# ddcr/shape_based_matching

Measured on AMD Instinct MI355X. Metric: templates*Mpixels/sec (whole Detector::match, frame resident in HBM), higher is better.
Workload: dtype u8; 1 GPU; case1 on MI355X: 1024x1024x3 frames x 360 templates per GPU (131/71 features), pyramid T={4,8}, threshold 90, 16 frame(s) per step, every frame's match list gathered to the host every step; stage=whole Detector::match per frame, templates_total=360, templates_per_gpu=360, parallelism=template-shard x1, frames_in_flight=64, input_buffers=8, exchange=none, n_ranks_seen=1, matches_distinct=8

## Files before the change

include/sbm.h:

```cpp
#ifndef SBM_H
#define SBM_H

#include <stdint.h>
#include "sbm_types.h"

#ifdef __cplusplus
extern "C" {
#endif

#define SBM_ABI_VERSION 1

typedef enum sbm_status {
    SBM_OK = 0,
    SBM_ERR_INVALID = -1,
    SBM_ERR_HIP = -2,
    SBM_ERR_CAPACITY = -3,
    SBM_ERR_STATE = -4
} sbm_status;

typedef struct sbm_ctx sbm_ctx;

typedef struct sbm_config {
    int32_t n_levels;
    int32_t T[SBM_MAX_LEVELS];
// ... 96 lines not shown
int64_t sbm_canonicalize(sbm_match_rec* recs, int64_t n);

typedef struct sbm_nms_params {
    float score_threshold;
    float nms_threshold;
    float eta;
    int32_t top_k;
} sbm_nms_params;
int sbm_nms_batch_device(sbm_ctx* ctx, const void* d_recs, const void* d_counts, int64_t cap, int32_t n_frames,
                         int32_t n_parts, int64_t part_stride, const sbm_nms_params* p, void* d_out, int64_t out_cap,
                         void* d_out_counts, void* stream);
int sbm_match_batch_host_end_nms(sbm_ctx* ctx, const sbm_nms_params* p, sbm_match_rec* out, int64_t out_cap, int32_t* counts);

int sbm_build_pyramid(sbm_ctx* ctx, const uint8_t* img_host, int32_t rows, int32_t cols,
                      int32_t stride, int32_t channels, const uint8_t* mask_host);
int sbm_set_quantized(sbm_ctx* ctx, int32_t level, const uint8_t* quantized_host, int32_t rows,
                      int32_t cols);
int sbm_get_quantized(sbm_ctx* ctx, int32_t level, uint8_t* out_host);
int sbm_get_quantized_frame(sbm_ctx* ctx, int32_t level, int32_t frame, uint8_t* out_host);
int sbm_get_linear_memories(sbm_ctx* ctx, int32_t level, uint8_t* out_host, int64_t cap_bytes,
                            int64_t* lm_stride);
int sbm_get_coarse_bitplanes(sbm_ctx* ctx, int32_t frame, uint8_t* out_host, int64_t cap_bytes);
int sbm_get_coarse_form(sbm_ctx* ctx, int32_t out[4]);
int sbm_level_dims(sbm_ctx* ctx, int32_t level, int32_t* rows, int32_t* cols);

int sbm_match_templates(sbm_ctx* ctx, float threshold, sbm_match_rec* out_host, int64_t cap,
                        int64_t* n_out);

int sbm_match_templates_device(sbm_ctx* ctx, float threshold, void* d_out, int64_t cap, void* d_count,
                               void* stream);


int sbm_quantized_orientations(sbm_ctx* ctx, const uint8_t* img_host, int32_t rows, int32_t cols,
                               int32_t stride, int32_t channels, float weak_threshold,
                               float* magnitude, uint8_t* angle, float* angle_ori);
int sbm_extract_local_maxima(sbm_ctx* ctx, const float* magnitude_host, const uint8_t* mask_host, int32_t rows, int32_t cols,
                             float strong_threshold, int32_t* xy, int64_t cap, int64_t* n_out);
int sbm_orientation_bins(sbm_ctx* ctx, const int16_t* gx, const int16_t* gy, int64_t n, uint8_t* q16);
int sbm_resize_linear(sbm_ctx* ctx, const uint8_t* img_host, int32_t rows, int32_t cols, int32_t stride, int32_t channels,
                      double fx, double fy, uint8_t* out, int64_t cap_bytes, int32_t* out_rows, int32_t* out_cols);
int sbm_pyrdown(sbm_ctx* ctx, const uint8_t* img_host, int32_t rows, int32_t cols, int32_t stride,
                int32_t channels, uint8_t* out_host);
int sbm_spread(sbm_ctx* ctx, const uint8_t* src_host, int32_t rows, int32_t cols, int32_t T,
               uint8_t* dst_host);
int sbm_compute_response_maps(sbm_ctx* ctx, const uint8_t* spread_host, int32_t rows, int32_t cols,
                              uint8_t* maps_host);
// ... 31 lines not shown
```

shape_based_matching_amd/capi.py:

```python
from __future__ import annotations

import ctypes as C
import os
from typing import List, Optional, Sequence, Tuple

import numpy as np

from .templates import FEATURE_DTYPE, LEVEL_DTYPE, MATCH_DTYPE, TemplateSet

TRAIN_FEATURE_DTYPE = np.dtype([("x", "<i4"), ("y", "<i4"), ("label", "<i4"), ("theta", "<f4")])

_HERE = os.path.dirname(os.path.abspath(__file__))
LIB_PATH = os.path.join(_HERE, "libsbm_hip.so")
SBM_MAX_LEVELS = 8

ABI_SYMBOLS = [
    "sbm_last_error", "sbm_abi_version", "sbm_create", "sbm_destroy", "sbm_upload_templates",
    "sbm_select_classes", "sbm_select_range", "sbm_match", "sbm_match_device", "sbm_match_batch_device", "sbm_canonicalize",
    "sbm_build_pyramid", "sbm_set_quantized", "sbm_get_quantized", "sbm_get_linear_memories",
    "sbm_level_dims", "sbm_match_templates", "sbm_quantized_orientations", "sbm_pyrdown", "sbm_spread",
    "sbm_compute_response_maps", "sbm_linearize", "sbm_similarity", "sbm_similarity_local",
    "sbm_set_profiling", "sbm_get_timings", "sbm_coarse_bytes", "sbm_get_stats",
    "sbm_set_result_mirror", "sbm_set_graph_mode", "sbm_set_quantize_mode", "sbm_resize_linear",
    "sbm_match_templates_device", "sbm_orientation_bins",
    "sbm_comm_unique_id", "sbm_comm_init", "sbm_comm_destroy", "sbm_match_device_sharded", "sbm_match_batch_device_sharded",
    "sbm_match_batch_device_banded", "sbm_pin_host_buffer", "sbm_unpin_host_buffer",
    "sbm_select_templates", "sbm_partition_templates", "sbm_match_sharded",
    "sbm_match_batch_host", "sbm_match_batch_host_begin", "sbm_match_batch_host_end", "sbm_extract_local_maxima",
    "sbm_train_batch", "sbm_train_batch_device",
    "sbm_set_pipeline_depth", "sbm_set_coarse_mode", "sbm_set_refine_order", "sbm_set_refine_bits", "sbm_get_coarse_bitplanes",
    "sbm_comm_count", "sbm_match_templates_device_sharded", "sbm_graph_count",
    "sbm_nms_batch_device", "sbm_match_batch_host_end_nms",
    "sbm_match_batch_device_masked", "sbm_match_batch_host_begin_masked", "sbm_match_batch_host_masked", "sbm_get_quantized_frame",
    "sbm_get_coarse_form",
]


class SbmConfig(C.Structure):
    _fields_ = [
        ("n_levels", C.c_int32),
        ("T", C.c_int32 * SBM_MAX_LEVELS),
        ("weak_threshold", C.c_float),
        ("device_id", C.c_int32),
        ("max_candidates", C.c_int64),
    ]


class SbmNmsParams(C.Structure):
    _fields_ = [
        ("score_threshold", C.c_float),
        ("nms_threshold", C.c_float),
        ("eta", C.c_float),
        ("top_k", C.c_int32),
    ]


class SbmError(RuntimeError):
# ... 84 lines not shown
    L.sbm_last_error.restype = C.c_char_p
    L.sbm_abi_version.restype = i32
    L.sbm_create.argtypes = [C.POINTER(SbmConfig), C.POINTER(vp)]
    L.sbm_destroy.argtypes = [vp]
    L.sbm_destroy.restype = None
    L.sbm_upload_templates.argtypes = [vp, i32, vp, vp, i64, vp, vp]
    L.sbm_select_classes.argtypes = [vp, vp, i32]
    L.sbm_select_range.argtypes = [vp, i32, i32]
    L.sbm_match.argtypes = [vp, vp, i32, i32, i32, i32, vp, f32, vp, i64, C.POINTER(i64)]
    L.sbm_match_device.argtypes = [vp, vp, i32, i32, i32, i32, vp, f32, vp, i64, vp, vp]
    L.sbm_match_batch_device.argtypes = [vp, vp, i64, i32, i32, i32, i32, i32, vp, f32, vp, i64, vp, vp]
    L.sbm_match_batch_device_masked.argtypes = [vp, vp, i64, i32, i32, i32, i32, i32, vp, i64, f32, vp, i64, vp, vp]
    L.sbm_match_batch_host_begin_masked.argtypes = [vp, vp, i32, i32, i32, i32, i32, vp, f32, i64, i32]
    L.sbm_match_batch_host_masked.argtypes = [vp, vp, i32, i32, i32, i32, i32, vp, f32, vp, i64, vp, i32]
    L.sbm_get_quantized_frame.argtypes = [vp, i32, i32, vp]
    L.sbm_canonicalize.argtypes = [vp, i64]
    L.sbm_canonicalize.restype = i64
    L.sbm_build_pyramid.argtypes = [vp, vp, i32, i32, i32, i32, vp]
    L.sbm_set_quantized.argtypes = [vp, i32, vp, i32, i32]
    L.sbm_get_quantized.argtypes = [vp, i32, vp]
    L.sbm_get_linear_memories.argtypes = [vp, i32, vp, i64, C.POINTER(i64)]
    L.sbm_get_coarse_bitplanes.argtypes = [vp, i32, vp, i64]
    L.sbm_get_coarse_form.argtypes = [vp, vp]
    L.sbm_level_dims.argtypes = [vp, i32, C.POINTER(i32), C.POINTER(i32)]
    L.sbm_match_templates.argtypes = [vp, f32, vp, i64, C.POINTER(i64)]
    L.sbm_quantized_orientations.argtypes = [vp, vp, i32, i32, i32, i32, f32, vp, vp, vp]
    L.sbm_pyrdown.argtypes = [vp, vp, i32, i32, i32, i32, vp]
    L.sbm_orientation_bins.argtypes = [vp, vp, vp, i64, vp]
    L.sbm_spread.argtypes = [vp, vp, i32, i32, i32, vp]
    L.sbm_compute_response_maps.argtypes = [vp, vp, i32, i32, vp]
    L.sbm_linearize.argtypes = [vp, vp, i32, i32, i32, vp]
    L.sbm_similarity.argtypes = [vp, i32, vp]
    L.sbm_similarity_local.argtypes = [vp, i32, i32, i32, i32, vp]
    L.sbm_set_profiling.argtypes = [vp, i32]
    L.sbm_get_timings.argtypes = [vp, vp, vp, i32, C.POINTER(i32)]
    L.sbm_coarse_bytes.argtypes = [vp, C.POINTER(i64)]
    L.sbm_get_stats.argtypes = [vp, C.POINTER(i64), C.POINTER(i64)]
    L.sbm_set_result_mirror.argtypes = [vp, vp, vp]
    L.sbm_set_graph_mode.argtypes = [vp, i32]
    L.sbm_graph_count.argtypes = [vp, C.POINTER(i32)]
    L.sbm_set_quantize_mode.argtypes = [vp, i32, i32]
    L.sbm_resize_linear.argtypes = [vp, vp, i32, i32, i32, i32, C.c_double, C.c_double, vp, i64, C.POINTER(i32), C.POINTER(i32)]
    L.sbm_match_templates_device.argtypes = [vp, f32, vp, i64, vp, vp]
    L.sbm_comm_unique_id.argtypes = [vp]
    L.sbm_comm_init.argtypes = [vp, i32, i32, vp]
    L.sbm_comm_count.argtypes = [vp, C.POINTER(i32)]
# ... 375 lines not shown
        out = np.empty((r, c), np.uint8)
        _check(lib().sbm_get_quantized_frame(self._h, level, frame, _p(out)))
        return out

    def get_linear_memories(self, level: int) -> np.ndarray:
        s = C.c_int64()
        _check(lib().sbm_get_linear_memories(self._h, level, None, 0, C.byref(s)))
        out = np.empty((8, s.value), np.uint8)
        _check(lib().sbm_get_linear_memories(self._h, level, _p(out), out.nbytes, C.byref(s)))
        return out

    def get_coarse_bitplanes(self, frame: int = 0) -> np.ndarray:
        s = C.c_int64()
        _check(lib().sbm_get_linear_memories(self._h, self.n_levels - 1, None, 0, C.byref(s)))
        out = np.empty((16, s.value // 8), np.uint8)
        _check(lib().sbm_get_coarse_bitplanes(self._h, frame, _p(out), out.nbytes))
        return out

    def coarse_form(self) -> Tuple[int, int, int, int]:
        out = np.zeros(4, np.int32)
        _check(lib().sbm_get_coarse_form(self._h, _p(out)))
        return tuple(int(v) for v in out)

    def match_templates(self, threshold: float) -> np.ndarray:
        out = np.empty(self._cap, MATCH_DTYPE)
        n = C.c_int64(0)
        _check(lib().sbm_match_templates(self._h, C.c_float(threshold), _p(out), self._cap, C.byref(n)))
        return out[: n.value].copy()

    def match_templates_device(self, threshold: float, d_out: int, cap: int, d_count: int, stream: int = 0):
        _check(lib().sbm_match_templates_device(self._h, C.c_float(threshold), C.c_void_p(d_out), cap, C.c_void_p(d_count),
                                                C.c_void_p(stream) if stream else None))

    def quantized_orientations(self, img: np.ndarray, weak: float, want_float: bool = True):
        img, r, c, ch = _img(img)
        ang = np.empty((r, c), np.uint8)
        mag = np.empty((r, c), np.float32) if want_float else None
        ori = np.empty((r, c), np.float32) if want_float else None
        _check(lib().sbm_quantized_orientations(self._h, _p(img), r, c, c * ch, ch, C.c_float(weak), _p(mag), _p(ang), _p(ori)))
        return mag, ang, ori

    def orientation_bins(self, gx: np.ndarray, gy: np.ndarray) -> np.ndarray:
        gx = np.ascontiguousarray(gx, np.int16)
        gy = np.ascontiguousarray(gy, np.int16)
        out = np.empty(gx.shape, np.uint8)
        _check(lib().sbm_orientation_bins(self._h, _p(gx), _p(gy), gx.size, _p(out)))
# ... 70 lines not shown
```

shape_based_matching_amd/csrc/sbm_capi.hip:

```cpp
#include <hip/hip_runtime.h>
#include <hip/hip_ext.h>
#include <dlfcn.h>

#include <algorithm>
#include <climits>
#include <cmath>
#include <cstdarg>
#include <cstdio>
#include <cstdlib>
#include <cstring>
#include <string>
#include <thread>
#include <vector>

#include "../../include/sbm.h"
#include "sbm_kernels.h"
#include "sbm_level_forms.h"
#include "sbm_quantize_stream.h"
#include "sbm_train_kernels.h"
#include "sbm_nms_kernels.h"

using namespace sbm;

#include "sbm_capi_ctx.inc"
#include "sbm_capi_match.inc"
#include "sbm_capi_stages.inc"
#include "sbm_capi_multi.inc"
#include "sbm_capi_nms.inc"
#include "sbm_capi_train.inc"
```

shape_based_matching_amd/csrc/sbm_capi_ctx.inc:

```
namespace {

thread_local std::string g_err;
void (*g_rccl_destroy_hook)(sbm_ctx*) = nullptr;

int fail(int code, const char* fmt, ...)
{
    char buf[512];
    va_list ap;
    va_start(ap, fmt);
    vsnprintf(buf, sizeof buf, fmt, ap);
    va_end(ap);
    g_err = buf;
    return code;
}

#define HIP_TRY(expr)                                                                              \
    do {                                                                                           \
        hipError_t e_ = (expr);                                                                    \
        if (e_ != hipSuccess)                                                                      \
            return fail(SBM_ERR_HIP, "%s failed: %s (%s:%d)", #expr, hipGetErrorString(e_), __FILE__, __LINE__); \
    } while (0)

struct DevBuf {
    void* p = nullptr;
// ... 26 lines not shown
    template <class T>
    T* as() const { return (T*)p; }
};

struct Timing {
    const char* name;
    hipEvent_t a, b;
    bool shared_a = false;
};

int64_t lm_stride_for(int rows, int cols, int T)
{
    int64_t W = cols / T, H = rows / T;
    int64_t s = (int64_t)T * T * W * H + W * H + 16 * W + 80;
    return (s + 63) / 64 * 64;
}

}

struct Tuning {
    int coarse = 0, quantize = 0, hs0 = 0, hs1 = 0, local_grid = 0, local_waves = 0, local_order = -1;
    bool qs_pack = true, full_lm = false, strip_lm = true, graph_fork = true, fused_bits = true, lm_allty = true;
    int bits_wide = -1, bits_dw = 0, bits_block = -1, match_bands = 0, local_bits = -1;
    bool sparse_strips = true, sparse_gradient = true;
    int src_hs = 0;
};
static const Tuning& tuning()
{
    static const Tuning t = [] {
        Tuning k;
        auto num = [](const char* name, int dflt) {
            const char* v = getenv(name);
            return v && *v ? atoi(v) : dflt;
        };
        if (const char* e = getenv("SBM_COARSE"))
            k.coarse = !strcmp(e, "block") ? 1 : (!strcmp(e, "wave") ? 2 : (!strcmp(e, "bits") ? 3 : (!strcmp(e, "bytes") ? 4 : 0)));
        if (const char* e = getenv("SBM_QUANTIZE")) k.quantize = !strcmp(e, "tile") ? 1 : (!strcmp(e, "stream") ? 2 : 0);
        if (const char* e = getenv("SBM_QS_HS")) {
            k.hs0 = atoi(e);
            k.hs1 = strchr(e, ',') ? atoi(strchr(e, ',') + 1) : k.hs0;
        }
        k.qs_pack = num("SBM_QS_PACK", 1) != 0;
        k.full_lm = num("SBM_FULL_LM", 0) != 0;
        k.strip_lm = num("SBM_STRIP_LM", 1) != 0;
        k.local_grid = std::max(0, num("SBM_LOCAL_GRID", 0));
        k.local_waves = num("SBM_LOCAL_WAVES", 0);
        k.local_order = num("SBM_LOCAL_ORDER", -1) == 2 ? 2 : num("SBM_LOCAL_ORDER", -1) == 0 ? 0 : -1;
        k.graph_fork = num("SBM_GRAPH_FORK", 1) != 0;
        k.fused_bits = num("SBM_FUSED_BITS", 1) != 0;
        k.bits_wide = num("SBM_BITS_WIDE", -1);
        k.lm_allty = num("SBM_LM_ALLTY", 1) != 0;
        k.bits_block = num("SBM_BITS_BLOCK", -1);
        k.local_bits = num("SBM_LOCAL_BITS", -1);
        k.sparse_strips = num("SBM_SPARSE_STRIPS", 1) != 0;
        k.sparse_gradient = k.sparse_strips && num("SBM_SPARSE_GRADIENT", 1) != 0;
        k.src_hs = std::min(4096, std::max(0, num("SBM_QS_SRC_HS", 0)));
        k.match_bands = std::min(8, std::max(0, num("SBM_MATCH_BANDS", 0)));
        k.bits_dw = num("SBM_BITS_DW", 0) == 2 ? 2 : (num("SBM_BITS_DW", 0) == 1 ? 1 : 0);
        return k;
    }();
    return t;
}

struct sbm_ctx {
    sbm_config cfg{};
    int n_simd = 1024;
    int L = 0;
    hipStream_t stream = nullptr;
    int64_t cand_cap = 0;

    int n_templates = 0;
    int64_t n_features = 0;
    std::vector<DevTL> h_tls;
    std::vector<uint32_t> h_fxy;
    std::vector<int32_t> h_class, h_tid;
    std::vector<int32_t> h_active;
    DevBuf d_tls, d_fxy, d_flabel, d_flevel, d_foff, d_class, d_tid, d_active, d_rawmin, d_rawkeep;
    DevBuf d_citems, d_cfoff, d_soff, d_soffbase;
    bool citems_dirty = true;
// ... 57 lines not shown
    DevBuf d_nms_labels, d_nms_scratch, d_nms_out;
    int32_t* h_nms_counts = nullptr;
    int h_nms_counts_frames = 0;
    DevBuf d_train, d_train_in, d_train_mask, d_train_out;

    struct GraphEntry {
        const void* img;
        int rows, cols, stride, ch;
        const void* mask;
        uint32_t thr_bits;
        void* out;
        int64_t cap;
        void* count;
        void* mo;
        void* mc;
        int frames;
        int64_t frame_stride;
        int64_t mask_stride;
        hipGraph_t graph;
        hipGraphExec_t exec;
        uint64_t last_use;
        bool sparse_grad = false;
        int32_t coarse_form[4] = {0, 0, 0, 0};
    };
    std::vector<GraphEntry> graphs;
    uint64_t graph_clock = 0;
    int quantize_mode = 0, quantize_hs = 0;
    int pipeline_depth = 1;
    int local_order = tuning().local_order;
    int32_t coarse_form[4] = {0, 0, 0, 0};
    void note_coarse_form(int kind, int P, bool wide, int dw)
    {
        coarse_form[0] = kind, coarse_form[1] = P, coarse_form[2] = wide ? 1 : 0, coarse_form[3] = dw;
    }
    int coarse_mode = tuning().coarse;
    int graph_pref = -1;
    bool auto_graph_off = false;
    int graph_captures_since_hit = 0;
    std::vector<GraphEntry> graph_seen;
    hipStream_t side = nullptr;
    hipEvent_t ev_fork[SBM_MAX_LEVELS] = {};
    hipEvent_t ev_join = nullptr;
    void drop_graphs()
    {
        for (auto& g : graphs) {
            (void)hipGraphExecDestroy(g.exec);
            (void)hipGraphDestroy(g.graph);
        }
        graphs.clear();
    }

    bool profiling = false;
    bool profiling_keep = false;
// ... 240 lines not shown
    int64_t keep_fs;
    const uint8_t* tile_flags;
    int n_tiles, T, W, H;
};

int source_pass_rows() { return tuning().src_hs > 0 ? (tuning().src_hs + 1) & ~1 : 32; }

int launch_quantize(sbm_ctx* c, hipStream_t s, const uint8_t* d_img, int rows, int cols, int stride, int ch,
                    const uint8_t* d_mask, float weak, uint8_t* d_out, float* d_mag, float* d_ori, uint8_t* d_pyr,
                    int frames = 1, int64_t img_fs = 0, int row_lo = 0, int row_hi = -1, bool tile_band = false, int64_t mask_fs = 0,
                    const QSForm* form = nullptr)
{
    if (!d_mask) mask_fs = 0;
    if (row_hi < 0) row_hi = rows;
    const bool band = row_lo > 0 || row_hi < rows;
    const int tile_row0 = tile_band ? row_lo / QT_R : 0;
    dim3 grid((cols + QT_C - 1) / QT_C, tile_band ? (row_hi - row_lo + QT_R - 1) / QT_R : (rows + QT_R - 1) / QT_R, frames);
    const float thr_sq = weak * weak;
    const bool wf = d_mag || d_ori;
    const int64_t out_fs = (int64_t)rows * cols, pyr_fs = (int64_t)(rows / 2) * (cols / 2) * ch;
    int hs = tile_band ? 0 : quantize_stream_rows(c, rows, cols, ch, frames, wf, img_fs, stride, band ? row_hi - row_lo : 0, mask_fs);
    if (form && (!hs || band || d_mask)) return fail(SBM_ERR_STATE, "a reduced gradient form needs a whole, unmasked launch of the streaming kernel");
    if (form && form->stage == QS_SOURCE) hs = source_pass_rows();
    if (hs) {
        QSArgs a;
        memset(&a, 0, sizeof a);
        a.img = d_img;
        a.mask = d_mask;
        a.out = d_out;
        a.pyr = d_pyr;
        a.img_fs = img_fs;
        a.out_fs = out_fs;
        a.pyr_fs = pyr_fs;
        a.mask_fs = mask_fs;
        a.rows = rows;
        a.cols = cols;
        a.stride = stride;
        a.thr_i = thr_sq < 2147483000.f ? (int)floorf(thr_sq) : INT_MAX;
        a.hs = hs;
        a.row_lo = row_lo;
        a.row_hi = row_hi;
        a.n_strips = (cols + QS_USEFUL - 1) / QS_USEFUL;
        a.n_rblocks = (row_hi - row_lo + hs - 1) / hs;
        a.frames = frames;
        a.pack_lanes = qs_pack_lanes(rows, cols, ch, frames, img_fs, stride, mask_fs);
        a.pack_groups = a.pack_lanes ? (frames + 64 / a.pack_lanes - 1) / (64 / a.pack_lanes) : 0;
        const int stage = form ? form->stage : (int)QS_WHOLE;
        if (stage == QS_SOURCE) {
            a.keep = form->keep;
            a.keep_fs = form->keep_fs;
        } else if (stage == QS_SPARSE) {
            a.pyr = nullptr;
            a.tile_flags = form->tile_flags;
            a.n_tiles = form->n_tiles;
            a.grid_t = form->T;
            a.grid_w = form->W;
            a.grid_h = form->H;
        }
        const dim3 g((unsigned)((quantize_stream_items(a) + 3) / 4));
#define SBM_QS(CH_)                                                                                                         \
        do {                                                                                                                \
            if (stage == QS_SOURCE) SBM_LAUNCH(c, "k_quantize", (k_quantize_stream<CH_, QS_SOURCE>), g, dim3(256), 0, s, a); \
            else if (stage == QS_SPARSE) SBM_LAUNCH(c, "k_quantize", (k_quantize_stream<CH_, QS_SPARSE>), g, dim3(256), 0, s, a); \
            else SBM_LAUNCH(c, "k_quantize", (k_quantize_stream<CH_, QS_WHOLE>), g, dim3(256), 0, s, a);                     \
        } while (0)
        if (ch == 1) SBM_QS(1);
        else SBM_QS(3);
#undef SBM_QS
        HIP_TRY(hipGetLastError());
        return 0;
    }
    if (band && !tile_band) return fail(SBM_ERR_INVALID, "a row band needs the streaming gradient kernel (cols %% 4 == 0, no float outputs)");
    if (tile_band && (row_lo % QT_R || (row_hi % QT_R && row_hi != rows))) return fail(SBM_ERR_INVALID, "a band of tiles must start and end on tile rows");
    const bool many = (int64_t)grid.x * grid.y * grid.z >= 2048;
#define SBM_QUANTIZE(CH_, WF_)                                                                                              \
    do {                                                                                                                    \
        if (many)                                                                                                           \
            SBM_LAUNCH(c, "k_quantize", (k_quantize<CH_, WF_, QN_THROUGHPUT>), grid, dim3(QN_THROUGHPUT), 0, s, d_img, rows, cols, \
                       stride, d_mask, thr_sq, d_out, d_mag, d_ori, d_pyr, img_fs, out_fs, pyr_fs, tile_row0, mask_fs);     \
        else                                                                                                                \
            SBM_LAUNCH(c, "k_quantize", (k_quantize<CH_, WF_, QN_LATENCY>), grid, dim3(QN_LATENCY), 0, s, d_img, rows, cols, stride, \
                       d_mask, thr_sq, d_out, d_mag, d_ori, d_pyr, img_fs, out_fs, pyr_fs, tile_row0, mask_fs);             \
    } while (0)
    if (ch == 1 && !wf) SBM_QUANTIZE(1, false);
    else if (ch == 1) SBM_QUANTIZE(1, true);
    else if (!wf) SBM_QUANTIZE(3, false);
    else SBM_QUANTIZE(3, true);
#undef SBM_QUANTIZE
    HIP_TRY(hipGetLastError());
    return 0;
}

// ... 264 lines not shown
        blocks += lma_level_blocks(W, H, sh);
        smem = std::max(smem, lma_lds_bytes(T, sh.cells, sh.grows));
    }
    if (blocks >= (int64_t)INT32_MAX) return fail(SBM_ERR_INVALID, "pyramid too large for one linear-memory launch");
    if (reset_count) {
        a.counters = c->d_counters.as<int32_t>();
        a.out_count = reset_count;
        c->counters_fresh = true;
    }
    SBM_LAUNCH(c, "k_build_lm", k_build_lm_any, dim3((unsigned)blocks, frames), dim3(LMA_THREADS), (size_t)smem, s, a);
    HIP_TRY(hipGetLastError());
    return 0;
}

int enqueue_pyramid(sbm_ctx* c, hipStream_t s, const uint8_t* d_img0, int stride0, const uint8_t* d_mask0,
                    int32_t* reset_count = nullptr, int frames = 1, int64_t img0_fs = 0, const Bands* bands = nullptr,
                    bool level0_gradient_done = false, int64_t mask0_fs = 0)
{
    const uint8_t* img = d_img0;
    int stride = stride0;
    const uint8_t* mask = d_mask0;
    int64_t mask_fs = d_mask0 ? mask0_fs : 0;
    c->last_frames = frames;
    const bool all_rows = all_rows_ok(c);
    c->counters_fresh = false;
    const PlanInputs pin = call_plan_inputs(c, d_mask0, stride0, frames, img0_fs, bands, level0_gradient_done);
    const BuildPlan plan = plan_build(pin, all_rows, reset_count != nullptr);
    if (!all_rows && frames > 1 && !pin.any_batch) {
        for (int l = 0; l < c->L; ++l)
            if (c->cfg.T[l] > LMA_MAX_T)
                return fail(SBM_ERR_INVALID, "batched match: level %d has T = %d, and a pyramid with a stride other than 4 or 8 or a level that is not "
                            "16-column-aligned batches up to T = %d only", l, c->cfg.T[l], LMA_MAX_T);
        return fail(SBM_ERR_STATE, "batched match: no linear-memory builder for this pyramid");
    }
    for (int l = 0; l < c->L; ++l) {
        const int nb = (l == 0 && level0_gradient_done) ? 0 : (bands && bands->n > 1 ? bands->count : 1);
        for (int b = 0; b < nb; ++b) {
            int lo = 0, hi = c->rows[l];
            if (bands && bands->n > 1) {
                const int br = c->rows[l] / bands->n, e = band_halo(c->L, l);
                lo = std::max(0, (bands->first + b) * br - e);
                hi = std::min(c->rows[l], (bands->first + b + 1) * br + e);
            }
            const int64_t img_fs = l == 0 ? img0_fs : (int64_t)c->rows[l] * c->cols[l] * c->channels;
            if (l == 0 && plan.sparse_gradient) {
                const QSForm form{QS_SOURCE, c->d_src0.as<uint8_t>(), (int64_t)c->rows[0] * c->cols[0] * c->channels, nullptr, 0, 0, 0, 0};
// ... 453 lines not shown
            }
            if (++c->graph_captures_since_hit > (int)(2 * GRAPH_CACHE)) {
                c->auto_graph_off = true;
                return 0;
            }
        }
        if (c->graphs.size() >= GRAPH_CACHE) {
            size_t lru = 0;
            for (size_t i = 1; i < c->graphs.size(); ++i)
                if (c->graphs[i].last_use < c->graphs[lru].last_use) lru = i;
            HIP_TRY(hipDeviceSynchronize());
            (void)hipGraphExecDestroy(c->graphs[lru].exec);
            (void)hipGraphDestroy(c->graphs[lru].graph);
            c->graphs.erase(c->graphs.begin() + lru);
        }
        sbm_ctx::GraphEntry ge = key;
        if (int e = capture(&ge.graph)) return e;
        hipError_t he = hipGraphInstantiate(&ge.exec, ge.graph, nullptr, nullptr, 0);
        if (he != hipSuccess) {
            (void)hipGraphDestroy(ge.graph);
            return fail(SBM_ERR_HIP, "hipGraphInstantiate failed: %s", hipGetErrorString(he));
        }
        memcpy(ge.coarse_form, c->coarse_form, sizeof ge.coarse_form);
        c->graphs.push_back(ge);
        hit = &c->graphs.back();
    } else {
        c->graph_captures_since_hit = 0;
    }
    hit->last_use = ++c->graph_clock;
    HIP_TRY(hipGraphLaunch(hit->exec, s));
    memcpy(c->coarse_form, hit->coarse_form, sizeof c->coarse_form);
    *launched = true;
    return 0;
}

int end_capture(hipStream_t m, int rc, hipGraph_t* graph)
{
    hipGraph_t g = nullptr;
    hipError_t e = hipStreamEndCapture(m, &g);
    if (rc) {
        if (g) (void)hipGraphDestroy(g);
        return rc;
    }
    if (e != hipSuccess || !g) return fail(SBM_ERR_HIP, "hipStreamEndCapture failed: %s", hipGetErrorString(e));
    *graph = g;
    return 0;
}

void record_match(sbm_ctx* c, bool one_launch, bool sparse_grad, bool any_batch)
{
    PlanInputs pin = plan_inputs(c);
    pin.any_batch = any_batch;
    record_match(c->forms, pin, one_launch, c->h_active.empty());
    c->levels_valid = c->L;
// ... 107 lines not shown
```

shape_based_matching_amd/csrc/sbm_capi_match.inc:

```
extern "C" {

const char* sbm_last_error(void) { return g_err.c_str(); }
int sbm_abi_version(void) { return SBM_ABI_VERSION; }

int sbm_create(const sbm_config* cfg, sbm_ctx** out)
{
    if (!cfg || !out) return fail(SBM_ERR_INVALID, "null argument");
    if (cfg->n_levels < 1 || cfg->n_levels > SBM_MAX_LEVELS) return fail(SBM_ERR_INVALID, "n_levels %d out of range", cfg->n_levels);
    for (int l = 0; l < cfg->n_levels; ++l)
        if (cfg->T[l] < 1 || cfg->T[l] > 64) return fail(SBM_ERR_INVALID, "T[%d]=%d out of range", l, cfg->T[l]);
    int ndev = 0;
    if (hipGetDeviceCount(&ndev) != hipSuccess || ndev <= 0)
        return fail(SBM_ERR_HIP, "no HIP device available: libsbm_hip has no CPU fallback");
    if (cfg->device_id < 0 || cfg->device_id >= ndev) return fail(SBM_ERR_INVALID, "device_id %d out of range (%d devices)", cfg->device_id, ndev);
    HIP_TRY(hipSetDevice(cfg->device_id));
    sbm_ctx* c = new sbm_ctx();
    c->cfg = *cfg;
    c->L = cfg->n_levels;
    {
        hipDeviceProp_t prop;
        if (hipGetDeviceProperties(&prop, cfg->device_id) == hipSuccess && prop.multiProcessorCount > 0) c->n_simd = 4 * prop.multiProcessorCount;
        else (void)hipGetLastError();
    }
    c->cand_cap = cfg->max_candidates > 0 ? cfg->max_candidates : (int64_t)1 << 20;
// ... 726 lines not shown
    return 0;
}

int sbm_get_coarse_bitplanes(sbm_ctx* c, int32_t frame, uint8_t* out, int64_t cap_bytes)
{
    if (!c || !out || frame < 0 || frame >= c->batch) return fail(SBM_ERR_INVALID, "bad argument");
    if (c->levels_valid < c->L) return fail(SBM_ERR_STATE, "pyramid not built");
    const int64_t need = 2 * c->lm_stride[c->L - 1];
    if (cap_bytes < need) return fail(SBM_ERR_CAPACITY, "need %lld bytes", (long long)need);
    HIP_TRY(hipSetDevice(c->cfg.device_id));
    HIP_TRY(hipDeviceSynchronize());
    if (!c->forms[c->L - 1].bit_planes || !c->d_blm.p) return fail(SBM_ERR_STATE, "the last call did not build the coarsest level's bit planes");
    HIP_TRY(hipMemcpy(out, c->d_blm.as<uint8_t>() + (size_t)frame * need, (size_t)need, hipMemcpyDeviceToHost));
    return 0;
}

int sbm_get_coarse_form(sbm_ctx* c, int32_t out[4])
{
    if (!c || !out) return fail(SBM_ERR_INVALID, "null argument");
    memcpy(out, c->coarse_form, sizeof c->coarse_form);
    return 0;
}

int sbm_level_dims(sbm_ctx* c, int32_t level, int32_t* rows, int32_t* cols)
{
    if (!c || level < 0 || level >= c->levels_valid) return fail(SBM_ERR_STATE, "level not resident");
    if (rows) *rows = c->rows[level];
    if (cols) *cols = c->cols[level];
    return 0;
}

int sbm_match_templates(sbm_ctx* c, float threshold, sbm_match_rec* out, int64_t cap, int64_t* n_out)
{
    if (!c || (!out && cap > 0) || !n_out) return fail(SBM_ERR_INVALID, "null argument");
    HIP_TRY(hipSetDevice(c->cfg.device_id));
    if (int e = order_after_caller_work(c)) return e;
    if (c->profiling && !c->profiling_keep) c->clear_timings();
    if (int e = enqueue_templates(c, c->stream, threshold, c->d_out.as<sbm_match_rec>(), c->cand_cap, c->d_outcount.as<int32_t>())) return e;
    int rc = fetch_results(c, c->stream, out, cap, n_out);
    if (c->profiling) collect_timings(c);
    return rc;
}
```

shape_based_matching_amd/csrc/sbm_wave_gfx950.h:

```cpp
#pragma once
#include <hip/hip_runtime.h>
#include <stdint.h>

namespace wv {

typedef uint32_t V;
typedef bool P;

typedef unsigned short wv_us2 __attribute__((ext_vector_type(2)));
typedef short wv_ss2 __attribute__((ext_vector_type(2)));
typedef uint32_t __attribute__((aligned(1))) wv_u32_unaligned;
typedef uint16_t __attribute__((aligned(1))) wv_u16_unaligned;

__device__ __forceinline__ V lane_id() { return __builtin_amdgcn_mbcnt_hi(~0u, __builtin_amdgcn_mbcnt_lo(~0u, 0u)); }
__device__ __forceinline__ V splat(uint32_t s) { return s; }

__device__ __forceinline__ V cold_splat(uint32_t s)
{
    V r;
    asm volatile("v_mov_b32 %0, %1" : "=v"(r) : "s"(s));
    return r;
}
__device__ __forceinline__ V dont_care()
{
    V r;
    asm volatile("" : "=v"(r));
    return r;
}

__device__ __forceinline__ V from_left(V x) { return (V)__builtin_amdgcn_mov_dpp((int)x, 0x138, 0xf, 0xf, true); }
__device__ __forceinline__ V from_right(V x) { return (V)__builtin_amdgcn_mov_dpp((int)x, 0x130, 0xf, 0xf, true); }
__device__ __forceinline__ uint32_t opaque(uint32_t k)
{
    asm("" : "+s"(k));
    return k;
}

__device__ __forceinline__ V perm(V hi, V lo, V sel) { return __builtin_amdgcn_perm(hi, lo, sel); }
__device__ __forceinline__ V alignbit(V hi, V lo, uint32_t sh) { return __builtin_amdgcn_alignbit(hi, lo, sh); }

__device__ __forceinline__ V udot2(V a, V b, V c)
{
    return __builtin_amdgcn_udot2(__builtin_bit_cast(wv_us2, a), __builtin_bit_cast(wv_us2, b), c, false);
}
__device__ __forceinline__ V sdot2(V a, V b, V c)
{
    return (V)__builtin_amdgcn_sdot2(__builtin_bit_cast(wv_ss2, a), __builtin_bit_cast(wv_ss2, b), (int)c, false);
}

__device__ __forceinline__ V sdot2_small(V a, V b)
{
    return (V)__builtin_amdgcn_sdot2(__builtin_bit_cast(wv_ss2, a), __builtin_bit_cast(wv_ss2, b), 0, true);
}

// ... 46 lines not shown
__device__ __forceinline__ V load_u32(const uint8_t* base, V off) { return *(const wv_u32_unaligned*)(base + off); }

struct Buf {
    __amdgpu_buffer_rsrc_t rsrc;
};
constexpr uint32_t BUF_DROP = 0x7ffffff0u;
__device__ __forceinline__ Buf make_buf(uint8_t* base, uint32_t bytes)
{
    Buf b;
    b.rsrc = __builtin_amdgcn_make_buffer_rsrc(base, 0, (int)bytes, 0x00020000);
    return b;
}
__device__ __forceinline__ void buf_store_u32(const Buf& b, V voff, uint32_t soff, V v) { __builtin_amdgcn_raw_buffer_store_b32(v, b.rsrc, (int)voff, (int)soff, 0); }
typedef uint32_t wv_u32x3 __attribute__((ext_vector_type(3)));
__device__ __forceinline__ void buf_store_u32_nt(const Buf& b, V voff, uint32_t soff, V v) { __builtin_amdgcn_raw_buffer_store_b32(v, b.rsrc, (int)voff, (int)soff, 2); }
__device__ __forceinline__ void buf_store_u32x3_nt(const Buf& b, V voff, uint32_t soff, V v0, V v1, V v2)
{
    __builtin_amdgcn_raw_buffer_store_b96(wv_u32x3{v0, v1, v2}, b.rsrc, (int)voff, (int)soff, 2);
}
__device__ __forceinline__ void buf_store_u16(const Buf& b, V voff, uint32_t soff, V v)
{
    __builtin_amdgcn_raw_buffer_store_b16((unsigned short)v, b.rsrc, (int)voff, (int)soff, 0);
}

}
```

Baseline: 71.07 million templates*Mpixels/s.

## Add wave-per-strip source-lines kernel for source copy and pyramid downsample

Adds a new kernel for the QS_SOURCE stage. Each wave owns a 256-pixel column strip over a block of rows. It streams rows through a 4-deep prefetch ring with wide buffer loads, writes the kept source copy with non-temporal stores, and computes the 5x5 Gaussian pyrDown in registers, using DPP neighbour exchange for strip edges. It replaces the generic streaming quantize kernel for that stage when alignment conditions hold, and is on by default. It also records which source form ran, exposed through a new getter. The aim is lower memory traffic and better load latency hiding, at the cost of a more complex, specialized code path.

```diff
diff --git a/include/sbm.h b/include/sbm.h
--- a/include/sbm.h
+++ b/include/sbm.h
@@ -142,6 +142,7 @@
                             int64_t* lm_stride);
 int sbm_get_coarse_bitplanes(sbm_ctx* ctx, int32_t frame, uint8_t* out_host, int64_t cap_bytes);
 int sbm_get_coarse_form(sbm_ctx* ctx, int32_t out[4]);
+int sbm_get_source_form(sbm_ctx* ctx, int32_t* out);
 int sbm_level_dims(sbm_ctx* ctx, int32_t level, int32_t* rows, int32_t* cols);
 
 int sbm_match_templates(sbm_ctx* ctx, float threshold, sbm_match_rec* out_host, int64_t cap,
diff --git a/shape_based_matching_amd/capi.py b/shape_based_matching_amd/capi.py
--- a/shape_based_matching_amd/capi.py
+++ b/shape_based_matching_amd/capi.py
@@ -33,6 +33,7 @@
     "sbm_nms_batch_device", "sbm_match_batch_host_end_nms",
     "sbm_match_batch_device_masked", "sbm_match_batch_host_begin_masked", "sbm_match_batch_host_masked", "sbm_get_quantized_frame",
     "sbm_get_coarse_form",
+    "sbm_get_source_form",
 ]
 
 
@@ -163,6 +164,7 @@
     L.sbm_get_linear_memories.argtypes = [vp, i32, vp, i64, C.POINTER(i64)]
     L.sbm_get_coarse_bitplanes.argtypes = [vp, i32, vp, i64]
     L.sbm_get_coarse_form.argtypes = [vp, vp]
+    L.sbm_get_source_form.argtypes = [vp, vp]
     L.sbm_level_dims.argtypes = [vp, i32, C.POINTER(i32), C.POINTER(i32)]
     L.sbm_match_templates.argtypes = [vp, f32, vp, i64, C.POINTER(i64)]
     L.sbm_quantized_orientations.argtypes = [vp, vp, i32, i32, i32, i32, f32, vp, vp, vp]
@@ -584,6 +586,11 @@
         _check(lib().sbm_get_coarse_form(self._h, _p(out)))
         return tuple(int(v) for v in out)
 
+    def source_form(self) -> int:
+        out = C.c_int32(0)
+        _check(lib().sbm_get_source_form(self._h, C.byref(out)))
+        return int(out.value)
+
     def match_templates(self, threshold: float) -> np.ndarray:
         out = np.empty(self._cap, MATCH_DTYPE)
         n = C.c_int64(0)
diff --git a/shape_based_matching_amd/csrc/sbm_capi.hip b/shape_based_matching_amd/csrc/sbm_capi.hip
--- a/shape_based_matching_amd/csrc/sbm_capi.hip
+++ b/shape_based_matching_amd/csrc/sbm_capi.hip
@@ -17,6 +17,7 @@
 #include "sbm_kernels.h"
 #include "sbm_level_forms.h"
 #include "sbm_quantize_stream.h"
+#include "sbm_source_lines.h"
 #include "sbm_train_kernels.h"
 #include "sbm_nms_kernels.h"
 
diff --git a/shape_based_matching_amd/csrc/sbm_capi_ctx.inc b/shape_based_matching_amd/csrc/sbm_capi_ctx.inc
--- a/shape_based_matching_amd/csrc/sbm_capi_ctx.inc
+++ b/shape_based_matching_amd/csrc/sbm_capi_ctx.inc
@@ -72,7 +72,7 @@
     int coarse = 0, quantize = 0, hs0 = 0, hs1 = 0, local_grid = 0, local_waves = 0, local_order = -1;
     bool qs_pack = true, full_lm = false, strip_lm = true, graph_fork = true, fused_bits = true, lm_allty = true;
     int bits_wide = -1, bits_dw = 0, bits_block = -1, match_bands = 0, local_bits = -1;
-    bool sparse_strips = true, sparse_gradient = true;
+    bool sparse_strips = true, sparse_gradient = true, source_lines = true;
     int src_hs = 0;
 };
 static const Tuning& tuning()
@@ -105,6 +105,7 @@
         k.sparse_strips = num("SBM_SPARSE_STRIPS", 1) != 0;
         k.sparse_gradient = k.sparse_strips && num("SBM_SPARSE_GRADIENT", 1) != 0;
         k.src_hs = std::min(4096, std::max(0, num("SBM_QS_SRC_HS", 0)));
+        k.source_lines = num("SBM_SOURCE_LINES", 1) != 0;
         k.match_bands = std::min(8, std::max(0, num("SBM_MATCH_BANDS", 0)));
         k.bits_dw = num("SBM_BITS_DW", 0) == 2 ? 2 : (num("SBM_BITS_DW", 0) == 1 ? 1 : 0);
         return k;
@@ -208,6 +209,7 @@
         uint64_t last_use;
         bool sparse_grad = false;
         int32_t coarse_form[4] = {0, 0, 0, 0};
+        int32_t source_form = 0;
     };
     std::vector<GraphEntry> graphs;
     uint64_t graph_clock = 0;
@@ -215,6 +217,7 @@
     int pipeline_depth = 1;
     int local_order = tuning().local_order;
     int32_t coarse_form[4] = {0, 0, 0, 0};
+    int32_t source_form = 0;
     void note_coarse_form(int kind, int P, bool wide, int dw)
     {
         coarse_form[0] = kind, coarse_form[1] = P, coarse_form[2] = wide ? 1 : 0, coarse_form[3] = dw;
@@ -501,6 +504,32 @@
     int hs = tile_band ? 0 : quantize_stream_rows(c, rows, cols, ch, frames, wf, img_fs, stride, band ? row_hi - row_lo : 0, mask_fs);
     if (form && (!hs || band || d_mask)) return fail(SBM_ERR_STATE, "a reduced gradient form needs a whole, unmasked launch of the streaming kernel");
     if (form && form->stage == QS_SOURCE) hs = source_pass_rows();
+    if (form && form->stage == QS_SOURCE && tuning().source_lines &&
+        source_lines_ok((uint64_t)(uintptr_t)d_img, stride, img_fs, frames, rows, cols, ch)) {
+        QSArgs a;
+        memset(&a, 0, sizeof a);
+        a.img = d_img;
+        a.pyr = d_pyr;
+        a.img_fs = img_fs;
+        a.pyr_fs = pyr_fs;
+        a.rows = rows;
+        a.cols = cols;
+        a.stride = stride;
+        a.hs = hs;
+        a.row_lo = 0;
+        a.row_hi = rows;
+        a.n_strips = sl_strips(cols);
+        a.n_rblocks = sl_row_blocks(0, rows, hs);
+        a.frames = frames;
+        a.keep = form->keep;
+        a.keep_fs = form->keep_fs;
+        const dim3 g((unsigned)((sl_items(cols, a.n_rblocks, frames) + 3) / 4));
+        if (ch == 1) SBM_LAUNCH(c, "k_quantize", (k_source_lines<1>), g, dim3(256), 0, s, a);
+        else SBM_LAUNCH(c, "k_quantize", (k_source_lines<3>), g, dim3(256), 0, s, a);
+        HIP_TRY(hipGetLastError());
+        c->source_form = 2;
+        return 0;
+    }
     if (hs) {
         QSArgs a;
         memset(&a, 0, sizeof a);
@@ -547,6 +576,7 @@
         else SBM_QS(3);
 #undef SBM_QS
         HIP_TRY(hipGetLastError());
+        if (stage == QS_SOURCE) c->source_form = 1;
         return 0;
     }
     if (band && !tile_band) return fail(SBM_ERR_INVALID, "a row band needs the streaming gradient kernel (cols %% 4 == 0, no float outputs)");
@@ -857,6 +887,7 @@
     const uint8_t* mask = d_mask0;
     int64_t mask_fs = d_mask0 ? mask0_fs : 0;
     c->last_frames = frames;
+    c->source_form = 0;
     const bool all_rows = all_rows_ok(c);
     c->counters_fresh = false;
     const PlanInputs pin = call_plan_inputs(c, d_mask0, stride0, frames, img0_fs, bands, level0_gradient_done);
@@ -1356,6 +1387,7 @@
             return fail(SBM_ERR_HIP, "hipGraphInstantiate failed: %s", hipGetErrorString(he));
         }
         memcpy(ge.coarse_form, c->coarse_form, sizeof ge.coarse_form);
+        ge.source_form = c->source_form;
         c->graphs.push_back(ge);
         hit = &c->graphs.back();
     } else {
@@ -1364,6 +1396,7 @@
     hit->last_use = ++c->graph_clock;
     HIP_TRY(hipGraphLaunch(hit->exec, s));
     memcpy(c->coarse_form, hit->coarse_form, sizeof c->coarse_form);
+    c->source_form = hit->source_form;
     *launched = true;
     return 0;
 }
diff --git a/shape_based_matching_amd/csrc/sbm_capi_match.inc b/shape_based_matching_amd/csrc/sbm_capi_match.inc
--- a/shape_based_matching_amd/csrc/sbm_capi_match.inc
+++ b/shape_based_matching_amd/csrc/sbm_capi_match.inc
@@ -772,6 +772,13 @@
     return 0;
 }
 
+int sbm_get_source_form(sbm_ctx* c, int32_t* out)
+{
+    if (!c || !out) return fail(SBM_ERR_INVALID, "null argument");
+    *out = c->source_form;
+    return 0;
+}
+
 int sbm_level_dims(sbm_ctx* c, int32_t level, int32_t* rows, int32_t* cols)
 {
     if (!c || level < 0 || level >= c->levels_valid) return fail(SBM_ERR_STATE, "level not resident");
diff --git a/shape_based_matching_amd/csrc/sbm_source_lines.h b/shape_based_matching_amd/csrc/sbm_source_lines.h
--- /dev/null
+++ b/shape_based_matching_amd/csrc/sbm_source_lines.h
@@ -0,0 +1,175 @@
+#pragma once
+#include "sbm_quantize_stream.h"
+#include "sbm_source_lines_plan.h"
+
+#ifdef SBM_WAVE_EMU
+namespace wv {
+inline V buf_load_dword(const Buf& b, const V& voff, uint32_t soff, uint32_t k, uint32_t n)
+{
+    V r;
+    for (int i = 0; i < WAVE; ++i) {
+        r.l[i] = 0;
+        if ((uint64_t)voff.l[i] + 4 * n > b.bytes) continue;
+        if ((uint64_t)voff.l[i] + soff + 4 * n > b.bytes || ((voff.l[i] + soff) & 3) || ((uintptr_t)b.base & 3)) __builtin_trap();
+        memcpy(&r.l[i], b.base + voff.l[i] + soff + 4 * k, 4);
+    }
+    return r;
+}
+inline void sched_fence() {}
+inline V buf_load_u32(const Buf& b, const V& voff, uint32_t soff) { return buf_load_dword(b, voff, soff, 0, 1); }
+inline void buf_load_u32x2(const Buf& b, const V& voff, uint32_t soff, V& v0, V& v1)
+{
+    v0 = buf_load_dword(b, voff, soff, 0, 2);
+    v1 = buf_load_dword(b, voff, soff, 1, 2);
+}
+inline void buf_load_u32x3(const Buf& b, const V& voff, uint32_t soff, V& v0, V& v1, V& v2)
+{
+    v0 = buf_load_dword(b, voff, soff, 0, 3);
+    v1 = buf_load_dword(b, voff, soff, 1, 3);
+    v2 = buf_load_dword(b, voff, soff, 2, 3);
+}
+inline void buf_store_u32x3(const Buf& b, const V& voff, uint32_t soff, const V& v0, const V& v1, const V& v2)
+{
+    V off = voff;
+    for (int i = 0; i < WAVE; ++i)
+        if ((uint64_t)voff.l[i] + 12 > b.bytes) off.l[i] = BUF_DROP;
+    buf_store_u32(b, off, soff, v0);
+    buf_store_u32(b, off, soff + 4, v1);
+    buf_store_u32(b, off, soff + 8, v2);
+}
+}
+#endif
+
+namespace sbm {
+
+constexpr int SL_PREFETCH = 4;
+
+template <int CH>
+__device__ __forceinline__ void source_lines_wave(const QSArgs& a, int strip, int rb, int frame)
+{
+    using namespace wv;
+    constexpr int ND = CH == 3 ? 3 : 1;
+    constexpr int NE = CH == 3 ? 2 : 1;
+    const int rows = a.rows, cols = a.cols;
+    const SlRows rr = sl_rows(rb, a.hs, a.row_lo, a.row_hi);
+    const int R0 = rr.r0, R1 = rr.r1, own0 = rr.own0;
+    const int drows = rows >> 1, dcols = cols >> 1;
+
+    const V lane = lane_id();
+    const V c0 = splat((uint32_t)(strip * SL_STRIP)) + (lane << 2);
+    const P in_img = lt_i(c0, splat((uint32_t)cols));
+    const V row_off = select(in_img, CH == 3 ? c0 + (c0 << 1) : c0, BUF_DROP);
+    const Buf src_buf = make_buf(const_cast<uint8_t*>(a.img) + (int64_t)frame * a.img_fs, sl_frame_bytes(rows, cols, CH, a.stride));
+    const Buf keep_buf = make_buf(a.keep + (int64_t)frame * a.keep_fs, (uint32_t)rows * (uint32_t)cols * CH);
+    const Buf pyr_buf = make_buf(a.pyr + (int64_t)frame * a.pyr_fs, (uint32_t)drows * (uint32_t)dcols * CH);
+    const V pyr_off = select(p_and(in_img, eq(lane & 1u, splat(0u))), CH == 3 ? (c0 >> 1) + ((c0 >> 1) << 1) : (c0 >> 1), BUF_DROP);
+    const P is_l0 = eq(lane, splat(0u)), is_l63 = eq(lane, splat(63u));
+    const int64_t e_left = sl_edge_left(strip, CH), e_right = sl_edge_right(strip, cols, CH);
+    const V edge_off = select(is_l0, e_left >= 0 ? (uint32_t)e_left : BUF_DROP, select(is_l63, e_right >= 0 ? (uint32_t)e_right : BUF_DROP, BUF_DROP));
+    const bool left_border = e_left < 0, right_border = e_right < 0;
+    const P first = eq(c0, splat(0u)), last = eq(c0, splat((uint32_t)(cols - 4)));
+    const uint32_t K4 = opaque(QS_K(4, 4));
+
+    V hw[6][CH];
+#pragma unroll
+    for (int k = 0; k < 6; ++k)
+#pragma unroll
+        for (int c = 0; c < CH; ++c) hw[k][c] = splat(0u);
+    V dq[6][ND], de[6][NE];
+    auto issue_load = [&](int i, V (&d)[ND], V (&e)[NE]) {
+        int y = R0 - 2 + i;
+        y = y < 0 ? 0 : (y > rows - 1 ? rows - 1 : y);
+        const uint32_t soff = (uint32_t)y * (uint32_t)a.stride;
+        if (CH == 3) {
+            buf_load_u32x2(src_buf, edge_off, soff, e[0], e[1 % NE]);
+            buf_load_u32x3(src_buf, row_off, soff, d[0], d[1 % ND], d[2 % ND]);
+        } else {
+            e[0] = buf_load_u32(src_buf, edge_off, soff);
+            d[0] = buf_load_u32(src_buf, row_off, soff);
+        }
+        sched_fence();
+    };
+    const int n_iter = R1 - R0 + 3;
+#pragma unroll
+    for (int p = 0; p < SL_PREFETCH; ++p) issue_load(p, dq[p], de[p]);
+    const int n_groups = (n_iter + 5) / 6;
+    for (int grp = 0; grp < n_groups; ++grp) {
+        const int i0 = grp * 6;
+#pragma unroll
+        for (int k = 0; k < 6; ++k) {
+            const int i = i0 + k, y = R0 - 2 + i;
+            issue_load(i + SL_PREFETCH, dq[(k + SL_PREFETCH) % 6], de[(k + SL_PREFETCH) % 6]);
+            const V d0 = dq[k][0], d1 = dq[k][1 % ND], d2 = dq[k][2 % ND], e0 = de[k][0], e1 = de[k][1 % NE];
+            const V koff = y >= own0 && y < R1 ? row_off : splat(BUF_DROP);
+            if (CH == 3) buf_store_u32x3_nt(keep_buf, koff, (uint32_t)(y * cols * CH), d0, d1, d2);
+            else buf_store_u32_nt(keep_buf, koff, (uint32_t)(y * cols * CH), d0);
+            if (CH == 3) {
+                V pd1 = select(is_l0, e0, from_left(d1)), pd2 = select(is_l0, e1, from_left(d2)), nd0 = select(is_l63, e0, from_right(d0));
+                if (left_border) {
+                    pd1 = select(first, d1, pd1);
+                    pd2 = select(first, perm(d2, perm(d1, d0, 0x0504030cu), 0x03020104u), pd2);
+                }
+                if (right_border) nd0 = select(last, perm(d2, d1, 0x0c040302u), nd0);
+                const V E[3] = {perm(d1, d0, 0x0c060c00u), perm(d1, d0, 0x0c070c01u), perm(d2, d0, 0x0c040c02u)};
+                const V O[3] = {perm(d2, d0, 0x0c050c03u), perm(d2, d1, 0x0c060c00u), perm(d2, d1, 0x0c070c01u)};
+                const V M2[3] = {perm(pd1, d0, 0x0c000c06u), perm(pd1, d0, 0x0c010c07u), perm(pd2, d0, 0x0c020c04u)};
+                const V M1[3] = {perm(pd2, d0, 0x0c030c05u), perm(pd2, d1, 0x0c000c06u), perm(pd2, d1, 0x0c010c07u)};
+                const V P2[3] = {perm(nd0, d1, 0x0c040c02u), perm(nd0, d1, 0x0c050c03u), perm(nd0, d2, 0x0c060c00u)};
+#pragma unroll
+                for (int c = 0; c < CH; ++c)
+                    hw[k][c] = pk_mad(E[c % 3], QS_K(6, 6), pk_mad(M1[c % 3] + O[c % 3], K4, M2[c % 3] + P2[c % 3]));
+            } else {
+                V pd = select(is_l0, e0, from_left(d0)), nd = select(is_l63, e0, from_right(d0));
+                if (left_border) pd = select(first, perm(d0, d0, 0x01020c0cu), pd);
+                if (right_border) nd = select(last, perm(d0, d0, 0x0c0c0c02u), nd);
+                const V E = perm(d0, d0, 0x0c020c00u), O = perm(d0, d0, 0x0c030c01u);
+                const V M2 = perm(pd, d0, 0x0c000c06u), M1 = perm(pd, d0, 0x0c010c07u), P2 = perm(nd, d0, 0x0c040c02u);
+                hw[k][0] = pk_mad(E, QS_K(6, 6), pk_mad(M1 + O, K4, M2 + P2));
+            }
+            sched_fence();
+            if ((k & 1) != 0) continue;
+            const int oy = (y - 2) >> 1;
+            const bool mine = oy >= (own0 >> 1) && oy < (R1 >> 1) && oy < drows;
+            const bool top = oy == 0, bot = !top && 2 * oy + 2 >= rows, two = top && rows == 2;
+            const uint32_t wr[5] = {top ? 0u : 1u, top ? 0u : 4u, two ? 8u : (bot ? 7u : 6u), top ? 8u : 4u, top ? (two ? 0u : 2u) : (bot ? 0u : 1u)};
+            V ob[CH];
+#pragma unroll
+            for (int c = 0; c < CH; ++c) {
+                V s = pk_mul(hw[(k + 2) % 6][c], wr[0] * 0x00010001u);
+#pragma unroll
+                for (int t = 1; t < 5; ++t) s = pk_mad(hw[(k + 2 + t) % 6][c], wr[t] * 0x00010001u, s);
+                ob[c] = pk_lshr(s + QS_K(128, 128), 8);
+            }
+            const V poff = mine ? pyr_off : splat(BUF_DROP);
+            const uint32_t prow = (uint32_t)(oy * dcols * CH);
+            if (CH == 3) {
+                const V A = perm(ob[2 % CH], perm(ob[1 % CH], ob[0], 0x020c0400u), 0x03040100u), B = perm(ob[2 % CH], ob[1 % CH], 0x0c0c0602u);
+                const V nA = from_right(A), nB = from_right(B);
+                buf_store_u32x3(pyr_buf, poff, prow, A, perm(nA, B, 0x05040100u), perm(nB, nA, 0x05040302u));
+            } else {
+                buf_store_u32(pyr_buf, poff, prow, perm(from_right(ob[0]), ob[0], 0x06040200u));
+            }
+            sched_fence();
+        }
+    }
+}
+
+template <int CH>
+__device__ __forceinline__ void source_lines_item(const QSArgs& a, int item)
+{
+    const int n_strips = sl_strips(a.cols);
+    if (item >= n_strips * a.n_rblocks * a.frames) return;
+    const SlItem it = sl_item(item, n_strips, a.frames);
+    source_lines_wave<CH>(a, it.strip, it.rb, it.frame);
+}
+
+#ifndef SBM_WAVE_EMU
+template <int CH>
+__global__ __launch_bounds__(256) void k_source_lines(const QSArgs a)
+{
+    const int item = (int)blockIdx.x * 4 + (int)__builtin_amdgcn_readfirstlane(threadIdx.x >> 6);
+    source_lines_item<CH>(a, item);
+}
+#endif
+
+}
diff --git a/shape_based_matching_amd/csrc/sbm_source_lines_plan.h b/shape_based_matching_amd/csrc/sbm_source_lines_plan.h
--- /dev/null
+++ b/shape_based_matching_amd/csrc/sbm_source_lines_plan.h
@@ -0,0 +1,62 @@
+#pragma once
+#include <stdint.h>
+
+#if defined(__HIPCC__) || defined(__CUDACC__)
+#define SBM_SL_HD __host__ __device__ __forceinline__
+#else
+#define SBM_SL_HD inline
+#endif
+
+namespace sbm {
+
+constexpr int SL_STRIP = 256;
+constexpr int SL_LANE_PX = 4;
+constexpr int64_t SL_MAX_FRAME_BYTES = 0x7ff00000ll;
+
+SBM_SL_HD bool source_lines_ok(uint64_t base, int64_t stride, int64_t frame_stride, int frames, int rows, int cols, int ch)
+{
+    if ((ch != 1 && ch != 3) || rows < 2 || (rows & 1) || cols < 64 || (cols & 63) || frames < 1) return false;
+    if (stride < (int64_t)cols * ch || (base & 3) || (stride & 3)) return false;
+    if (frames > 1 && (frame_stride & 3)) return false;
+    return (rows - 1) * stride + (int64_t)cols * ch < SL_MAX_FRAME_BYTES;
+}
+
+SBM_SL_HD uint32_t sl_frame_bytes(int rows, int cols, int ch, int stride) { return (uint32_t)((int64_t)(rows - 1) * stride + (int64_t)cols * ch); }
+
+SBM_SL_HD int sl_strips(int cols) { return (cols + SL_STRIP - 1) / SL_STRIP; }
+SBM_SL_HD int sl_row_blocks(int row_lo, int row_hi, int hs) { return (row_hi - row_lo + hs - 1) / hs; }
+SBM_SL_HD int sl_items(int cols, int n_rblocks, int frames) { return sl_strips(cols) * n_rblocks * frames; }
+
+struct SlItem {
+    int strip, rb, frame;
+};
+SBM_SL_HD SlItem sl_item(int item, int n_strips, int frames)
+{
+    const int per_rb = n_strips * frames, rb = item / per_rb, r = item - rb * per_rb;
+    return SlItem{r % n_strips, rb, r / n_strips};
+}
+
+struct SlRows {
+    int r0, r1, own0;
+};
+SBM_SL_HD SlRows sl_rows(int rb, int hs, int row_lo, int row_hi)
+{
+    SlRows r;
+    r.own0 = row_lo + rb * hs;
+    r.r0 = r.own0;
+    if (r.r0 + hs > row_hi) r.r0 = row_hi - row_lo > hs ? row_hi - hs : row_lo;
+    r.r1 = r.r0 + hs < row_hi ? r.r0 + hs : row_hi;
+    return r;
+}
+
+SBM_SL_HD int sl_lane_col(int strip, int lane) { return strip * SL_STRIP + lane * SL_LANE_PX; }
+SBM_SL_HD int64_t sl_row_off(int strip, int lane, int cols, int ch) { return sl_lane_col(strip, lane) < cols ? (int64_t)sl_lane_col(strip, lane) * ch : -1; }
+SBM_SL_HD int64_t sl_pyr_off(int strip, int lane, int cols, int ch)
+{
+    return (lane & 1) == 0 && sl_lane_col(strip, lane) < cols ? (int64_t)(sl_lane_col(strip, lane) >> 1) * ch : -1;
+}
+SBM_SL_HD int sl_edge_bytes(int ch) { return ch == 3 ? 8 : 4; }
+SBM_SL_HD int64_t sl_edge_left(int strip, int ch) { return strip > 0 ? (int64_t)strip * SL_STRIP * ch - sl_edge_bytes(ch) : -1; }
+SBM_SL_HD int64_t sl_edge_right(int strip, int cols, int ch) { return (strip + 1) * SL_STRIP < cols ? (int64_t)(strip + 1) * SL_STRIP * ch : -1; }
+
+}
diff --git a/shape_based_matching_amd/csrc/sbm_wave_gfx950.h b/shape_based_matching_amd/csrc/sbm_wave_gfx950.h
--- a/shape_based_matching_amd/csrc/sbm_wave_gfx950.h
+++ b/shape_based_matching_amd/csrc/sbm_wave_gfx950.h
@@ -30,6 +30,7 @@
 
 __device__ __forceinline__ V from_left(V x) { return (V)__builtin_amdgcn_mov_dpp((int)x, 0x138, 0xf, 0xf, true); }
 __device__ __forceinline__ V from_right(V x) { return (V)__builtin_amdgcn_mov_dpp((int)x, 0x130, 0xf, 0xf, true); }
+__device__ __forceinline__ void sched_fence() { __builtin_amdgcn_sched_barrier(0); }
 __device__ __forceinline__ uint32_t opaque(uint32_t k)
 {
     asm("" : "+s"(k));
@@ -122,5 +123,22 @@
 {
     __builtin_amdgcn_raw_buffer_store_b16((unsigned short)v, b.rsrc, (int)voff, (int)soff, 0);
 }
+__device__ __forceinline__ void buf_store_u32x3(const Buf& b, V voff, uint32_t soff, V v0, V v1, V v2)
+{
+    __builtin_amdgcn_raw_buffer_store_b96(wv_u32x3{v0, v1, v2}, b.rsrc, (int)voff, (int)soff, 0);
+}
+
+typedef uint32_t wv_u32x2 __attribute__((ext_vector_type(2)));
+__device__ __forceinline__ V buf_load_u32(const Buf& b, V voff, uint32_t soff) { return __builtin_amdgcn_raw_buffer_load_b32(b.rsrc, (int)voff, (int)soff, 0); }
+__device__ __forceinline__ void buf_load_u32x2(const Buf& b, V voff, uint32_t soff, V& v0, V& v1)
+{
+    const wv_u32x2 r = __builtin_amdgcn_raw_buffer_load_b64(b.rsrc, (int)voff, (int)soff, 0);
+    v0 = r.x, v1 = r.y;
+}
+__device__ __forceinline__ void buf_load_u32x3(const Buf& b, V voff, uint32_t soff, V& v0, V& v1, V& v2)
+{
+    const wv_u32x3 r = __builtin_amdgcn_raw_buffer_load_b96(b.rsrc, (int)voff, (int)soff, 0);
+    v0 = r.x, v1 = r.y, v2 = r.z;
+}
 
 }
```

Measured after the change: 73.74 million templates*Mpixels/s (median of 6 runs). 1.04x the previous value.
